# Roboy/gym-roboy

Measured on AMD Instinct MI355X. Metric: env-steps/sec, MsjRobot (3-DOF/8-tendon) batched rollout, higher is better.
Workload: dtype f32

## Files before the change

gym_roboy_amd/csrc/msj_kernels.hpp:

```cpp
#pragma once
#include "rtc_compat.hpp"
#include "msj_math.hpp"
#include "philox.hpp"
#include "env_common.hpp"

#if defined(RB_JIT_TABLE)
namespace rbk { __device__ constexpr rb::MsjConst<float, 8> BAKED = RB_JIT_TABLE; }
#else
#include "msj_baked.hpp"
#endif

namespace rbk {

using rbe::EnvParams;
using rbe::GoalBox;
using rbe::goal_value;
using rbe::mul_then_add;

constexpr int NT8 = 8;
constexpr int RS = rb::MsjModel<float, 8>::RS;
using Const8 = rb::MsjConst<float, NT8>;
constexpr int NTX = 16;
using ConstX = rb::MsjConst<float, NTX>;


template <bool BK, typename CONST>
__device__ __forceinline__ const CONST &robot_consts(const CONST &kernarg) {
    if constexpr (BK) return rbk::BAKED; else return kernarg;
}

struct SpLds {
    const float *col;
    int stride;
    __device__ __forceinline__ float operator()(int k) const { return col[k * stride]; }
};

struct Scale8 { float v[NT8]; };

template <int INTEG, int BLOCK, int UNROLL, bool BK = false>
__global__ void __launch_bounds__(BLOCK)
msj_step_env_per_lane(const Const8 c_arg, float *__restrict__ q, float *__restrict__ qd,
                      uint32_t *__restrict__ feas, const float *__restrict__ act, const Scale8 us, long n, long cnt) {
    const Const8 &c = robot_consts<BK>(c_arg);
    const long i = long(blockIdx.x) * BLOCK + threadIdx.x;
    if (i >= cnt) return;
    float qq[3], vv[3], sp[NT8];
    const float4 a0 = reinterpret_cast<const float4 *>(act)[2 * i];
    const float4 a1 = reinterpret_cast<const float4 *>(act)[2 * i + 1];
#pragma unroll
    for (int j = 0; j < 3; ++j) { qq[j] = q[j * n + i]; vv[j] = qd[j * n + i]; }
    const float a[NT8] = {a0.x, a0.y, a0.z, a0.w, a1.x, a1.y, a1.z, a1.w};
#pragma unroll
    for (int k = 0; k < NT8; ++k) sp[k] = a[k] * us.v[k];
    bool ok;
    if (UNROLL >= NT8) {
        ok = rb::MsjModel<float, NT8>::template step_sp<INTEG, UNROLL>(c, qq, vv, rb::SpArray<float, NT8>{sp});
    } else {
        __shared__ float lds_sp[NT8][BLOCK];
#pragma unroll
        for (int k = 0; k < NT8; ++k) lds_sp[k][threadIdx.x] = sp[k];
        ok = rb::MsjModel<float, NT8>::template step_sp<INTEG, UNROLL>(c, qq, vv, SpLds{&lds_sp[0][threadIdx.x], BLOCK});
    }
#pragma unroll
    for (int j = 0; j < 3; ++j) { q[j * n + i] = qq[j]; qd[j * n + i] = vv[j]; }
    feas[i] = ok ? 1u : 0u;
}




__device__ __forceinline__ __amdgpu_buffer_rsrc_t wg_rsrc(const void *base, int bytes) {
    return __builtin_amdgcn_make_buffer_rsrc(const_cast<void *>(base), 0, bytes, 0x00020000);
}

template <int INTEG, int BLOCK, bool BK = false>
__global__ void __launch_bounds__(BLOCK)
msj_step_env_per_lane_rs(const Const8 c_arg, float *__restrict__ q, float *__restrict__ qd,
                         uint32_t *__restrict__ feas, const float *__restrict__ act, const Scale8 us, long n, long cnt) {
    const Const8 &c = robot_consts<BK>(c_arg);
    const long env0 = long(blockIdx.x) * BLOCK;
    const long left = cnt - env0;
    const int live = int(left < BLOCK ? left : BLOCK);
    const int le = int(threadIdx.x);
    if (le >= live) return;
    const int off = le * 4;
    float qq[3], vv[3], u[NT8];
    const __amdgpu_buffer_rsrc_t ra = wg_rsrc(act + env0 * NT8, live * NT8 * 4);
    typedef float f4 __attribute__((ext_vector_type(4)));
    const f4 a0 = __builtin_bit_cast(f4, __builtin_amdgcn_raw_buffer_load_b128(ra, off * NT8, 0, 0));
    const f4 a1 = __builtin_bit_cast(f4, __builtin_amdgcn_raw_buffer_load_b128(ra, off * NT8 + 16, 0, 0));
#pragma unroll
    for (int j = 0; j < 3; ++j) {
        qq[j] = __uint_as_float(__builtin_amdgcn_raw_buffer_load_b32(wg_rsrc(q + j * n + env0, live * 4), off, 0, 0));
        vv[j] = __uint_as_float(__builtin_amdgcn_raw_buffer_load_b32(wg_rsrc(qd + j * n + env0, live * 4), off, 0, 0));
    }
    const float a[NT8] = {a0.x, a0.y, a0.z, a0.w, a1.x, a1.y, a1.z, a1.w};
#pragma unroll
    for (int k = 0; k < NT8; ++k) u[k] = a[k] * us.v[k];
    const bool ok = rb::MsjModel<float, NT8>::template step_rs<INTEG>(c, qq, vv, u);
#pragma unroll
    for (int j = 0; j < 3; ++j) {
        __builtin_amdgcn_raw_buffer_store_b32(__float_as_uint(qq[j]), wg_rsrc(q + j * n + env0, live * 4), off, 0, 0);
        __builtin_amdgcn_raw_buffer_store_b32(__float_as_uint(vv[j]), wg_rsrc(qd + j * n + env0, live * 4), off, 0, 0);
    }
    __builtin_amdgcn_raw_buffer_store_b32(ok ? 1u : 0u, wg_rsrc(feas + env0, live * 4), off, 0, 0);
}


struct PairMap { int a[4], d[4]; };
struct Scale4 { float v[4]; };

template <int CTRL>
__device__ __forceinline__ float rbk_dpp(float v) {
    return __int_as_float(__builtin_amdgcn_update_dpp(0, __float_as_int(v), CTRL, 0xF, 0xF, true));
}

template <int MIRROR>
struct AccelMirrorHalf {
    const Const8 &c;
    const float *u;
    __device__ __forceinline__ void operator()(const float q[3], const float qd[3], float qdd[3]) const {
        using M = rb::MsjModel<float, NT8>;
        const M::Frame f = M::frame(q, qd);
        float tx, ty, tz;
        M::half_torque(c, f, u, tx, ty, tz);
        M::template mirror_combine<MIRROR>(tx, ty, tz, rbk_dpp<0xB1>(tx), rbk_dpp<0xB1>(ty), rbk_dpp<0xB1>(tz));
        M::rigid_body(c, f, qd, tx, ty, tz, qdd);
    }
};

template <int INTEG, int BLOCK, int MIRROR, bool BK = false>
__global__ void __launch_bounds__(BLOCK)
msj_step_mirror_pairs(const Const8 c_arg, const PairMap pm, float *__restrict__ q, float *__restrict__ qd,
                      uint32_t *__restrict__ feas, const float *__restrict__ act, const Scale4 us, long n, long cnt) {
    const Const8 &c = robot_consts<BK>(c_arg);
    const long env0 = long(blockIdx.x) * (BLOCK / 2);
    const long left = cnt - env0;
    const int live = int(left < BLOCK / 2 ? left : BLOCK / 2);
    const int le = int(threadIdx.x >> 1);
    if (le >= live) return;
    const bool odd = (threadIdx.x & 1) != 0;
    const int off = le * 4, oddi = int(threadIdx.x & 1);
    float qq[3], vv[3], u[4];
    const __amdgpu_buffer_rsrc_t ra = wg_rsrc(act + env0 * NT8, live * NT8 * 4);
#pragma unroll
    for (int k = 0; k < 4; ++k) u[k] = __uint_as_float(__builtin_amdgcn_raw_buffer_load_b32(ra, off * NT8 + pm.a[k] + oddi * pm.d[k], 0, 0)) * us.v[k];
#pragma unroll
    for (int j = 0; j < 3; ++j) {
        qq[j] = __uint_as_float(__builtin_amdgcn_raw_buffer_load_b32(wg_rsrc(q + j * n + env0, live * 4), off, 0, 0));
        vv[j] = __uint_as_float(__builtin_amdgcn_raw_buffer_load_b32(wg_rsrc(qd + j * n + env0, live * 4), off, 0, 0));
    }
    constexpr int F0 = MIRROR == 0 ? 0 : 1, F1 = 2;
    const uint32_t flip = odd ? 0x80000000u : 0u;
    qq[F0] = __uint_as_float(__float_as_uint(qq[F0]) ^ flip); vv[F0] = __uint_as_float(__float_as_uint(vv[F0]) ^ flip);
    qq[F1] = __uint_as_float(__float_as_uint(qq[F1]) ^ flip); vv[F1] = __uint_as_float(__float_as_uint(vv[F1]) ^ flip);
    const bool ok = rb::MsjModel<float, NT8>::template integrate_acc<INTEG>(c, qq, vv, AccelMirrorHalf<MIRROR>{c, u});
    const int soff = odd ? 0x7fffff00 : le * 4;
#pragma unroll
    for (int j = 0; j < 3; ++j) {
        __builtin_amdgcn_raw_buffer_store_b32(__float_as_uint(qq[j]), wg_rsrc(q + j * n + env0, live * 4), soff, 0, 0);
        __builtin_amdgcn_raw_buffer_store_b32(__float_as_uint(vv[j]), wg_rsrc(qd + j * n + env0, live * 4), soff, 0, 0);
    }
    __builtin_amdgcn_raw_buffer_store_b32(ok ? 1u : 0u, wg_rsrc(feas + env0, live * 4), soff, 0, 0);
}


template <int INTEG, int BLOCK, int UNROLL, bool BK = false>
__global__ void __launch_bounds__(BLOCK)
msj_rollout_fused(const Const8 c_arg, float *__restrict__ q, float *__restrict__ qd, uint32_t *__restrict__ feas,
                  const float *__restrict__ act_ring, int ring, int n_steps, const Scale8 us, long n) {
    const Const8 &c = robot_consts<BK>(c_arg);
    const long i = long(blockIdx.x) * BLOCK + threadIdx.x;
    if (i >= n) return;
    float qq[3], vv[3];
#pragma unroll
    for (int j = 0; j < 3; ++j) { qq[j] = q[j * n + i]; vv[j] = qd[j * n + i]; }
    bool ok = true;
    const float4 *rec = reinterpret_cast<const float4 *>(act_ring) + 2 * i;
    float4 a0 = rec[0], a1 = rec[1];
    __shared__ float lds_sp[UNROLL >= NT8 ? 1 : NT8][BLOCK];
    int slab = 0;
    for (int t = 0; t < n_steps; ++t) {
        const float a[NT8] = {a0.x, a0.y, a0.z, a0.w, a1.x, a1.y, a1.z, a1.w};
        float sp[NT8];
#pragma unroll
        for (int k = 0; k < NT8; ++k) sp[k] = a[k] * us.v[k];
        if (t + 1 < n_steps) {
            slab = slab + 1 == ring ? 0 : slab + 1;
            const float4 *nx = rec + long(slab) * 2 * n;
            a0 = nx[0]; a1 = nx[1];
        }
        if (UNROLL == RS) {
            ok = rb::MsjModel<float, NT8>::template step_rs<INTEG>(c, qq, vv, sp);
        } else if (UNROLL >= NT8) {
            ok = rb::MsjModel<float, NT8>::template step_sp<INTEG, UNROLL>(c, qq, vv, rb::SpArray<float, NT8>{sp});
        } else {
#pragma unroll
            for (int k = 0; k < NT8; ++k) lds_sp[k][threadIdx.x] = sp[k];
            ok = rb::MsjModel<float, NT8>::template step_sp<INTEG, UNROLL>(c, qq, vv, SpLds{&lds_sp[0][threadIdx.x], BLOCK});
        }
    }
#pragma unroll
    for (int j = 0; j < 3; ++j) { q[j * n + i] = qq[j]; qd[j * n + i] = vv[j]; }
    feas[i] = ok ? 1u : 0u;
}



__device__ __forceinline__ void draw_goal3(const float (&lo)[3], const float (&hi)[3], uint64_t seed, uint64_t gid, uint32_t draw, float g[3]) {
    const rb::Philox4 r = rb::philox_draw(seed, gid, draw, rb::STREAM_GOALS, 0u);
#pragma unroll
    for (int j = 0; j < 3; ++j) g[j] = goal_value(lo[j], hi[j], r.v[j]);
}
__device__ __forceinline__ void draw_goal3(const GoalBox &box, uint64_t seed, uint64_t gid, uint32_t draw, float g[3]) {
    const float lo[3] = {box.lo[0], box.lo[1], box.lo[2]}, hi[3] = {box.hi[0], box.hi[1], box.hi[2]};
    draw_goal3(lo, hi, seed, gid, draw, g);
}

struct MsjEnvArgs {
    EnvParams e;
    float box_lo[3], box_hi[3];
    float *q, *qd;
    uint32_t *feas;
    float *goal;
    uint32_t *step_num;
    float *ep_ret;
    uint32_t *goal_count;
    const float *act;
    float *obs, *reward;
    uint32_t *done;
    double *ep_sum;
    uint32_t *ep_cnt, *infeas_n;
    long n, cnt;
    uint64_t seed, env0;
};
__host__ __device__ constexpr int msj_env_args_offset(int lead) { return (lead + int(alignof(MsjEnvArgs)) - 1) / int(alignof(MsjEnvArgs)) * int(alignof(MsjEnvArgs)); }
typedef const __attribute__((address_space(4))) MsjEnvArgs *msj_env_kernarg_ptr;
__device__ __forceinline__ msj_env_kernarg_ptr late_env_args(int offset) {
    const __attribute__((address_space(4))) char *p = (const __attribute__((address_space(4))) char *)__builtin_amdgcn_kernarg_segment_ptr();
    asm volatile("" : "+s"(p));
    return (msj_env_kernarg_ptr)(p + offset);
}

struct NoDoneHook {
    __device__ __forceinline__ void operator()(long, uint64_t, uint64_t, int) const {}
};

template <typename ARGS, typename HOOK = NoDoneHook>
__device__ __forceinline__ void env_account(ARGS a, long i, float (&qq)[3], float (&vv)[3], float (&gg)[3], bool ok,
                                            const HOOK &on_done = HOOK{}) {
    EnvParams e;
    e.vel_penalty = a->e.vel_penalty; e.bonus = a->e.bonus; e.max_len = a->e.max_len; e.auto_reset = a->e.auto_reset;
    e.penalty = a->e.penalty; e.bonus_val = a->e.bonus_val;
    e.a_lo = a->e.a_lo; e.a_hi = a->e.a_hi; e.v_lo = a->e.v_lo; e.v_hi = a->e.v_hi;
    e.act_hi = a->e.act_hi; e.slope = a->e.slope; e.tol_a2 = a->e.tol_a2; e.tol_v2 = a->e.tol_v2;
    e.a_scale = a->e.a_scale; e.v_scale = a->e.v_scale;
    const long n = a->n;
    float *__restrict__ q = a->q, *__restrict__ qd = a->qd, *__restrict__ goal = a->goal, *__restrict__ ep_ret = a->ep_ret;
    float *__restrict__ obs = a->obs, *__restrict__ reward = a->reward;
    uint32_t *__restrict__ feas = a->feas, *__restrict__ step_num = a->step_num, *__restrict__ goal_count = a->goal_count;
    uint32_t *__restrict__ done = a->done, *__restrict__ ep_cnt = a->ep_cnt, *__restrict__ infeas_n = a->infeas_n;
    double *__restrict__ ep_sum = a->ep_sum;
    uint32_t sn = step_num[i] + 1u;

    float dq2 = 0.0f, dv2 = 0.0f;
#pragma unroll
    for (int j = 0; j < 3; ++j) {
        const float dq = qq[j] - gg[j];
        dq2 += dq * dq;
        dv2 += vv[j] * vv[j];
    }
    bool reached;
    float r = rbe::env_reward(e, dq2, dv2, ok, reached);
    const bool dn = reached || (sn > uint32_t(e.max_len));

    float o[9] = {qq[0], qq[1], qq[2], vv[0], vv[1], vv[2], gg[0], gg[1], gg[2]};
    float ret = ep_ret[i] + r;
    uint32_t fz = ok ? 1u : 0u;
    if (!ok) infeas_n[i] += 1u;
    if (dn) {
        rbe::stat_add(&ep_sum[i], double(ret)); rbe::stat_add(&ep_sum[n + i], double(ret) * double(ret));
        rbe::stat_add(&ep_cnt[i], 1u); rbe::stat_add(&ep_cnt[n + i], sn - 1u); rbe::stat_add(&ep_cnt[2 * n + i], reached ? 1u : 0u);
        const uint64_t gid = a->env0 + uint64_t(i);
        const uint64_t seed = a->seed;
        const float lo[3] = {a->box_lo[0], a->box_lo[1], a->box_lo[2]}, hi[3] = {a->box_hi[0], a->box_hi[1], a->box_hi[2]};
        uint32_t draw = goal_count[i];
        draw_goal3(lo, hi, seed, gid, draw + (e.auto_reset ? 1u : 0u), gg);
        on_done(i, gid, seed, e.auto_reset);
        draw += e.auto_reset ? 2u : 1u;
        if (e.auto_reset) {
#pragma unroll
            for (int j = 0; j < 3; ++j) { qq[j] = 0.0f; vv[j] = 0.0f; o[j] = 0.0f; o[3 + j] = 0.0f; o[6 + j] = gg[j]; }
            sn = 1u; fz = 1u;
        }
        ret = 0.0f;
        goal_count[i] = draw;
#pragma unroll
        for (int j = 0; j < 3; ++j) goal[j * n + i] = gg[j];
    }
#pragma unroll
    for (int j = 0; j < 3; ++j) { q[j * n + i] = qq[j]; qd[j * n + i] = vv[j]; }
    feas[i] = fz; step_num[i] = sn; ep_ret[i] = ret;
    typedef float f4u __attribute__((ext_vector_type(4), aligned(4)));
    float *orow = obs + i * 9;
    *reinterpret_cast<f4u *>(orow) = f4u{o[0], o[1], o[2], o[3]};
    *reinterpret_cast<f4u *>(orow + 4) = f4u{o[4], o[5], o[6], o[7]};
    orow[8] = o[8];
    reward[i] = r; done[i] = dn ? 1u : 0u;
}

template <int INTEG, int BLOCK, int UNROLL, typename CONST = Const8, bool BK = false>
__global__ void __launch_bounds__(BLOCK)
msj_env_step_kernel(const CONST c_arg, const MsjEnvArgs a) {
    const float *__restrict__ q = a.q, *__restrict__ qd = a.qd, *__restrict__ goal = a.goal, *__restrict__ act = a.act;
    const long n = a.n, cnt = a.cnt;
    const float slope = a.e.slope, act_hi = a.e.act_hi;
    const CONST &c = robot_consts<BK>(c_arg);
    const long i = long(blockIdx.x) * BLOCK + threadIdx.x;
    if (i >= cnt) return;
    float qq[3], vv[3], gg[3];
#pragma unroll
    for (int j = 0; j < 3; ++j) { qq[j] = q[j * n + i]; vv[j] = qd[j * n + i]; gg[j] = goal[j * n + i]; }
    auto rescale = [&](float x) { return mul_then_add(slope, fminf(fmaxf(x, -1.0f), 1.0f) - 1.0f, act_hi); };
    bool ok;
    if constexpr (UNROLL == 0) {
        __shared__ float lds_sp[NTX][BLOCK];
        const int nt = c.nt;
        const float *row = act + i * nt;
        for (int k = 0; k < nt; ++k) lds_sp[k][threadIdx.x] = rescale(row[k]) * c.ten[k].ksg;
        ok = rb::MsjModel<float, NTX>::template step_sp<INTEG, 0>(c, qq, vv, SpLds{&lds_sp[0][threadIdx.x], BLOCK});
    } else {
    float sp[NT8];
    const float4 a0 = reinterpret_cast<const float4 *>(act)[2 * i];
    const float4 a1 = reinterpret_cast<const float4 *>(act)[2 * i + 1];
    const float av[NT8] = {a0.x, a0.y, a0.z, a0.w, a1.x, a1.y, a1.z, a1.w};
#pragma unroll
    for (int k = 0; k < NT8; ++k) sp[k] = rescale(av[k]) * c.ten[k].ksg;
    if (UNROLL == RS) {
        ok = rb::MsjModel<float, NT8>::template step_rs<INTEG>(c, qq, vv, sp);
    } else if (UNROLL >= NT8) {
        ok = rb::MsjModel<float, NT8>::template step_sp<INTEG, UNROLL>(c, qq, vv, rb::SpArray<float, NT8>{sp});
    } else {
        __shared__ float lds_sp[NT8][BLOCK];
#pragma unroll
        for (int k = 0; k < NT8; ++k) lds_sp[k][threadIdx.x] = sp[k];
        ok = rb::MsjModel<float, NT8>::template step_sp<INTEG, UNROLL>(c, qq, vv, SpLds{&lds_sp[0][threadIdx.x], BLOCK});
    }
    }
    if constexpr (BK) env_account(&a, i, qq, vv, gg, ok);
    else env_account(late_env_args(msj_env_args_offset(int(sizeof(CONST)))), i, qq, vv, gg, ok);
}


template <int INTEG, int BLOCK, int MIRROR, bool BK = false>
__global__ void __launch_bounds__(BLOCK)
msj_env_step_mirror_pairs(const Const8 c_arg, const PairMap pm, const MsjEnvArgs a) {
    const float *__restrict__ q = a.q, *__restrict__ qd = a.qd, *__restrict__ goal = a.goal, *__restrict__ act = a.act;
    const long n = a.n, cnt = a.cnt;
    const float slope = a.e.slope, act_hi = a.e.act_hi;
    const Const8 &c = robot_consts<BK>(c_arg);
    const long wg0 = long(blockIdx.x) * (BLOCK / 2);
    const long left = cnt - wg0;
    const int live = int(left < BLOCK / 2 ? left : BLOCK / 2);
    const int le = int(threadIdx.x >> 1);
    if (le >= live) return;
    const bool odd = (threadIdx.x & 1) != 0;
    const int off = le * 4, oddi = int(threadIdx.x & 1);
    const long i = wg0 + le;
    float qq[3], vv[3], gg[3], u[4];
    const __amdgpu_buffer_rsrc_t ra = wg_rsrc(act + wg0 * NT8, live * NT8 * 4);
#pragma unroll
    for (int k = 0; k < 4; ++k) {
        const float x = __uint_as_float(__builtin_amdgcn_raw_buffer_load_b32(ra, off * NT8 + pm.a[k] + oddi * pm.d[k], 0, 0));
        u[k] = mul_then_add(slope, fminf(fmaxf(x, -1.0f), 1.0f) - 1.0f, act_hi) * c.ten[k].ksg;
    }
#pragma unroll
    for (int j = 0; j < 3; ++j) {
        qq[j] = __uint_as_float(__builtin_amdgcn_raw_buffer_load_b32(wg_rsrc(q + j * n + wg0, live * 4), off, 0, 0));
        vv[j] = __uint_as_float(__builtin_amdgcn_raw_buffer_load_b32(wg_rsrc(qd + j * n + wg0, live * 4), off, 0, 0));
        gg[j] = __uint_as_float(__builtin_amdgcn_raw_buffer_load_b32(wg_rsrc(goal + j * n + wg0, live * 4), off, 0, 0));
    }
    constexpr int F0 = MIRROR == 0 ? 0 : 1, F1 = 2;
    const uint32_t flip = odd ? 0x80000000u : 0u;
    qq[F0] = __uint_as_float(__float_as_uint(qq[F0]) ^ flip); vv[F0] = __uint_as_float(__float_as_uint(vv[F0]) ^ flip);
    qq[F1] = __uint_as_float(__float_as_uint(qq[F1]) ^ flip); vv[F1] = __uint_as_float(__float_as_uint(vv[F1]) ^ flip);
    const bool ok = rb::MsjModel<float, NT8>::template integrate_acc<INTEG>(c, qq, vv, AccelMirrorHalf<MIRROR>{c, u});
    if (odd) return;
    if constexpr (BK) env_account(&a, i, qq, vv, gg, ok);
    else env_account(late_env_args(msj_env_args_offset(int(sizeof(Const8) + sizeof(PairMap)))), i, qq, vv, gg, ok);
}


}
```

gym_roboy_amd/csrc/msj_math.hpp:

```cpp
#pragma once
#include "rtc_compat.hpp"

#if defined(__HIPCC__)
#define RB_HD __host__ __device__ __forceinline__
#else
#define RB_HD inline
#endif


namespace rb {

template <typename T> struct Fast;
template <> struct Fast<double> {
    static RB_HD void sincos(double x, double &s, double &c) { s = ::sin(x); c = ::cos(x); }
    static RB_HD double exp(double x) { return ::exp(x); }
    static RB_HD double exp2(double x) { return ::exp2(x); }
    static RB_HD double rsqrt(double x) { return 1.0 / ::sqrt(x); }
    static RB_HD double rcp(double x) { return 1.0 / x; }
};
template <> struct Fast<float> {
    static RB_HD void sincos(float x, float &s, float &c) {
#if defined(__HIP_DEVICE_COMPILE__)
        s = __sinf(x); c = __cosf(x);
#else
        s = ::sinf(x); c = ::cosf(x);
#endif
    }
    static RB_HD float exp(float x) {
#if defined(__HIP_DEVICE_COMPILE__)
        return __expf(x);
#else
        return ::expf(x);
#endif
    }
    static RB_HD float exp2(float x) {
#if defined(__HIP_DEVICE_COMPILE__)
        return __builtin_amdgcn_exp2f(x);
#else
        return ::exp2f(x);
#endif
    }
    static RB_HD float rsqrt(float x) {
#if defined(__HIP_DEVICE_COMPILE__)
        return __builtin_amdgcn_rsqf(x);
#else
        return 1.0f / ::sqrtf(x);
#endif
    }
    static RB_HD float rcp(float x) {
#if defined(__HIP_DEVICE_COMPILE__)
        return __builtin_amdgcn_rcpf(x);
#else
        return 1.0f / x;
#endif
    }
};

template <typename T> RB_HD T tmin(T a, T b) {
#if defined(__HIP_DEVICE_COMPILE__)
    if constexpr (std::is_same<T, float>::value) return __builtin_fminf(a, b);
#endif
    return a < b ? a : b;
}
template <typename T> RB_HD T tmax(T a, T b) {
#if defined(__HIP_DEVICE_COMPILE__)
    if constexpr (std::is_same<T, float>::value) return __builtin_fmaxf(a, b);
#endif
    return a > b ? a : b;
}
template <typename T> RB_HD T tclamp(T x, T lo, T hi) {
#if defined(__HIP_DEVICE_COMPILE__)
    if constexpr (std::is_same<T, float>::value) return __builtin_amdgcn_fmed3f(x, lo, hi);
#endif
    return tmin(tmax(x, lo), hi);
}

template <typename T>
struct alignas(64) MsjTendon {
    T A[3];
    T Bv[3];
    T B2[3];
    T ab2;
    T il0s;
    T elcs;
    T ksg;
    T fmaxv;
    T pad[2];
};

template <typename T>
struct TendonUnits {
    T lc;
    T vl0;
    T fmax;
    T pad;
};

template <typename T>
struct TendonReading { T length, rate, activation, force; };

template <typename T, int NT>
struct MsjConst {
    MsjTendon<T> ten[NT];
    T IO[6];
    T mc[3];
    T g[3];
    T arm[3], damp[3], qlo[3], qhi[3], qdmax[3];
    T kps;
    T pe_k2s;
    T inv_pe_den;
    T fv_c1l, fv_c2l;
    T fv_c2s;
    T fv_k;
    T h;
    int32_t nsub;
    int32_t simple;
    int32_t nt;
};

template <typename T, int NT>
struct SpArray {
    const T *v;
    RB_HD T operator()(int k) const { return v[k]; }
};

struct NominalBody {
    template <typename T> RB_HD T mass(T x) const { return x; }
    template <typename T> RB_HD T damping(int, T x) const { return x; }
};

template <typename T, int NT>
struct MsjModel {
    using C = MsjConst<T, NT>;

    struct Frame {
        T s0, c0, s1, c1, s2, c2;
        T r00, r01, r02, r10, r11, r12, r20, r21, r22;
        T wx, wy, wz;
    };

    static RB_HD Frame frame(const T q[3], const T qd[3]) {
        Frame f;
        Fast<T>::sincos(q[0], f.s0, f.c0);
        Fast<T>::sincos(q[1], f.s1, f.c1);
        Fast<T>::sincos(q[2], f.s2, f.c2);
        f.r00 = f.c1 * f.c2; f.r01 = -f.c1 * f.s2; f.r02 = f.s1;
        f.r10 = f.c0 * f.s2 + f.s0 * f.s1 * f.c2; f.r11 = f.c0 * f.c2 - f.s0 * f.s1 * f.s2; f.r12 = -f.s0 * f.c1;
        f.r20 = f.s0 * f.s2 - f.c0 * f.s1 * f.c2; f.r21 = f.s0 * f.c2 + f.c0 * f.s1 * f.s2; f.r22 = f.c0 * f.c1;
        f.wx = f.r00 * qd[0] + f.s2 * qd[1];
        f.wy = f.r01 * qd[0] + f.c2 * qd[1];
        f.wz = f.r02 * qd[0] + qd[2];
        return f;
    }

    static RB_HD void tendon(const C &c, const Frame &f, const MsjTendon<T> &t, T u, T &tx, T &ty, T &tz) {
        const T ax = f.r00 * t.A[0] + f.r10 * t.A[1] + f.r20 * t.A[2];
        const T ay = f.r01 * t.A[0] + f.r11 * t.A[1] + f.r21 * t.A[2];
        const T az = f.r02 * t.A[0] + f.r12 * t.A[1] + f.r22 * t.A[2];
        const T d2 = ax * t.B2[0] + (ay * t.B2[1] + (az * t.B2[2] + t.ab2));
        const T mx = ay * t.Bv[2] - az * t.Bv[1];
        const T my = az * t.Bv[0] - ax * t.Bv[2];
        const T mz = ax * t.Bv[1] - ay * t.Bv[0];
        tendon_force(c, f, t, u, d2, mx, my, mz, tx, ty, tz);
    }

    static RB_HD void tendon_force(const C &c, const Frame &f, const MsjTendon<T> &t, T u, T d2, T mx, T my, T mz,
                                   T &tx, T &ty, T &tz) {
        const T inv = Fast<T>::rsqrt(d2);
        const T v = (f.wx * mx + f.wy * my + f.wz * mz) * inv;
        const T es = (d2 * inv) * t.il0s + t.elcs;
        const T act = tclamp(c.kps * es - u, T(0), T(1));
        const T fl = Fast<T>::exp2(-(es * es));
        const T vp = tmax(v, T(0)), p = tclamp(v + T(1), T(0), T(1));
        const T num = c.fv_c1l * vp + p;
        const T den = c.fv_c2l * vp + (c.fv_c2s * p + c.fv_k);
        const T rden = Fast<T>::rcp(den);
        const T fpe = tmax(Fast<T>::exp2(c.pe_k2s * es) * c.inv_pe_den - c.inv_pe_den, T(0));
        const T Fs = (t.fmaxv * inv) * ((act * fl) * num * rden + fpe);
        tx -= Fs * mx; ty -= Fs * my; tz -= Fs * mz;
    }

    static RB_HD TendonReading<T> tendon_state(const C &c, const Frame &f, const MsjTendon<T> &t, const TendonUnits<T> &pu, T u) {
        const T ax = f.r00 * t.A[0] + f.r10 * t.A[1] + f.r20 * t.A[2];
        const T ay = f.r01 * t.A[0] + f.r11 * t.A[1] + f.r21 * t.A[2];
        const T az = f.r02 * t.A[0] + f.r12 * t.A[1] + f.r22 * t.A[2];
        const T d2 = ax * t.B2[0] + (ay * t.B2[1] + (az * t.B2[2] + t.ab2));
        const T mx = ay * t.Bv[2] - az * t.Bv[1];
        const T my = az * t.Bv[0] - ax * t.Bv[2];
        const T mz = ax * t.Bv[1] - ay * t.Bv[0];
        const T inv = Fast<T>::rsqrt(d2);
        const T v = (f.wx * mx + f.wy * my + f.wz * mz) * inv;
        const T dl = d2 * inv;
        const T es = dl * t.il0s + t.elcs;
        const T act = tclamp(c.kps * es - u, T(0), T(1));
        const T fl = Fast<T>::exp2(-(es * es));
        const T vp = tmax(v, T(0)), p = tclamp(v + T(1), T(0), T(1));
        const T num = c.fv_c1l * vp + p;
        const T den = c.fv_c2l * vp + (c.fv_c2s * p + c.fv_k);
        const T rden = Fast<T>::rcp(den);
        const T fpe = tmax(Fast<T>::exp2(c.pe_k2s * es) * c.inv_pe_den - c.inv_pe_den, T(0));
        TendonReading<T> r;
        r.length = dl + pu.lc;
        r.rate = v * pu.vl0;
        r.activation = act;
        r.force = pu.fmax * ((act * fl) * num * rden + fpe);
        return r;
    }

    static RB_HD MsjTendon<T> scaled_tendon(const MsjTendon<T> &t, T fscale) {
        MsjTendon<T> s = t;
        s.fmaxv = t.fmaxv * fscale;
        return s;
    }

    static RB_HD T prescale(const C &c, int k, T setpoint) { return c.ten[k].ksg * setpoint; }

    template <typename BP> static RB_HD T bmass(const BP *bp, T x) {
        if constexpr (std::is_same<BP, NominalBody>::value) return x; else return bp->mass(x);
    }
    template <typename BP> static RB_HD T bdamp(const BP *bp, int j, T x) {
        if constexpr (std::is_same<BP, NominalBody>::value) return x; else return bp->damping(j, x);
    }
    template <typename BP = NominalBody>
    static RB_HD void rigid_body(const C &c, const Frame &f, const T qd[3], T tx, T ty, T tz, T qdd[3], const BP *bp = nullptr) {
        const T r00 = f.r00, r01 = f.r01, r02 = f.r02, s2 = f.s2, c2 = f.c2;
        const T Ixx = bmass(bp, c.IO[0]), Iyy = bmass(bp, c.IO[1]), Izz = bmass(bp, c.IO[2]);
        const T z0x = -f.s1 * c2 * qd[1] - f.c1 * s2 * qd[2];
        const T z0y = f.s1 * s2 * qd[1] - f.c1 * c2 * qd[2];
        const T z0z = f.c1 * qd[1];
        const T bx = z0x * qd[0] + c2 * qd[2] * qd[1];
        const T by = z0y * qd[0] - s2 * qd[2] * qd[1];
        const T bz = z0z * qd[0];
        T m00, m01, m02, m11, m12, m22, vx, vy, vz;
        if (c.simple) {
            const T a0x = Ixx * r00, a0y = Iyy * r01, a0z = Izz * r02;
            const T a1x = Ixx * s2, a1y = Iyy * c2;
            m00 = r00 * a0x + r01 * a0y + r02 * a0z + c.arm[0];
            m01 = s2 * a0x + c2 * a0y;
            m02 = a0z;
            m11 = s2 * a1x + c2 * a1y + c.arm[1];
            m12 = T(0);
            m22 = Izz + c.arm[2];
            const T hx = Ixx * f.wx, hy = Iyy * f.wy, hz = Izz * f.wz;
            const T nx = Ixx * bx + (f.wy * hz - f.wz * hy);
            const T ny = Iyy * by + (f.wz * hx - f.wx * hz);
            const T nz = Izz * bz + (f.wx * hy - f.wy * hx);
            const T k = bmass(bp, c.mc[2]) * c.g[2];
            vx = tx - k * f.r21 - nx;
            vy = ty + k * f.r20 - ny;
            vz = tz - nz;
        } else {
            const T Ixy = bmass(bp, c.IO[3]), Ixz = bmass(bp, c.IO[4]), Iyz = bmass(bp, c.IO[5]);
            const T a0x = Ixx * r00 + Ixy * r01 + Ixz * r02;
            const T a0y = Ixy * r00 + Iyy * r01 + Iyz * r02;
            const T a0z = Ixz * r00 + Iyz * r01 + Izz * r02;
            const T a1x = Ixx * s2 + Ixy * c2;
            const T a1y = Ixy * s2 + Iyy * c2;
            const T a1z = Ixz * s2 + Iyz * c2;
            m00 = r00 * a0x + r01 * a0y + r02 * a0z + c.arm[0];
            m01 = s2 * a0x + c2 * a0y;
            m02 = a0z;
            m11 = s2 * a1x + c2 * a1y + c.arm[1];
            m12 = a1z;
            m22 = Izz + c.arm[2];
            const T hx = a0x * qd[0] + a1x * qd[1] + Ixz * qd[2];
            const T hy = a0y * qd[0] + a1y * qd[1] + Iyz * qd[2];
            const T hz = a0z * qd[0] + a1z * qd[1] + Izz * qd[2];
            const T nx = Ixx * bx + Ixy * by + Ixz * bz + (f.wy * hz - f.wz * hy);
            const T ny = Ixy * bx + Iyy * by + Iyz * bz + (f.wz * hx - f.wx * hz);
            const T nz = Ixz * bx + Iyz * by + Izz * bz + (f.wx * hy - f.wy * hx);
            const T gx = r00 * c.g[0] + f.r10 * c.g[1] + f.r20 * c.g[2];
            const T gy = r01 * c.g[0] + f.r11 * c.g[1] + f.r21 * c.g[2];
            const T gz = r02 * c.g[0] + f.r12 * c.g[1] + f.r22 * c.g[2];
            vx = tx + (bmass(bp, c.mc[1]) * gz - bmass(bp, c.mc[2]) * gy) - nx;
            vy = ty + (bmass(bp, c.mc[2]) * gx - bmass(bp, c.mc[0]) * gz) - ny;
            vz = tz + (bmass(bp, c.mc[0]) * gy - bmass(bp, c.mc[1]) * gx) - nz;
        }
        const T t0 = r00 * vx + r01 * vy + r02 * vz - bdamp(bp, 0, c.damp[0]) * qd[0];
        const T t1 = s2 * vx + c2 * vy - bdamp(bp, 1, c.damp[1]) * qd[1];
        const T t2 = vz - bdamp(bp, 2, c.damp[2]) * qd[2];
        const T k00 = m11 * m22 - m12 * m12;
        const T k01 = m02 * m12 - m01 * m22;
        const T k02 = m01 * m12 - m02 * m11;
        const T k11 = m00 * m22 - m02 * m02;
        const T k12 = m01 * m02 - m00 * m12;
        const T k22 = m00 * m11 - m01 * m01;
        const T idet = Fast<T>::rcp(m00 * k00 + m01 * k01 + m02 * k02);
        qdd[0] = (k00 * t0 + k01 * t1 + k02 * t2) * idet;
        qdd[1] = (k01 * t0 + k11 * t1 + k12 * t2) * idet;
        qdd[2] = (k02 * t0 + k12 * t1 + k22 * t2) * idet;
    }

    template <int UNROLL, typename SP>
    struct AccelAllTendons {
        const C &c;
        const SP &sp;
        RB_HD void operator()(const T q[3], const T qd[3], T qdd[3]) const {
            const Frame f = frame(q, qd);
            T tx = T(0), ty = T(0), tz = T(0);
            if (UNROLL == 0) {
#pragma unroll 1
                for (int k = 0; k < c.nt; ++k) tendon(c, f, c.ten[k], sp(k), tx, ty, tz);
            } else {
                constexpr int U = UNROLL > 0 ? UNROLL : 1;
#pragma unroll U
                for (int k = 0; k < NT; ++k) tendon(c, f, c.ten[k], sp(k), tx, ty, tz);
            }
            rigid_body(c, f, qd, tx, ty, tz, qdd);
        }
    };

    template <int MIRROR> static RB_HD T mirror_sign(int j) { return (j == 2 || j == MIRROR) ? T(-1) : T(1); }
    static RB_HD void half_torque(const C &c, const Frame &f, const T u[4], T &tx, T &ty, T &tz) {
        tx = T(0); ty = T(0); tz = T(0);
#pragma unroll
        for (int k = 0; k < 4; ++k) {
            tendon(c, f, c.ten[k], u[k], tx, ty, tz);
#if defined(__HIP_DEVICE_COMPILE__)
            __builtin_amdgcn_sched_barrier(0);
#endif
        }
    }
    template <int MIRROR>
    static RB_HD void mirror_combine(T &tx, T &ty, T &tz, T px, T py, T pz) {
        tx = MIRROR == 0 ? tx - px : tx + px;
        ty = MIRROR == 0 ? ty + py : ty - py;
        tz = tz - pz;
    }

    static RB_HD void sat(const C &c, const T v[3], T out[3]) {
#pragma unroll
        for (int j = 0; j < 3; ++j) out[j] = tclamp(v[j], -c.qdmax[j], c.qdmax[j]);
    }

    static RB_HD bool limit(const C &c, T q[3], T qd[3]) {
        bool ok = true;
#pragma unroll
        for (int j = 0; j < 3; ++j) {
            const bool over = q[j] > c.qhi[j], under = q[j] < c.qlo[j];
            qd[j] = tclamp(qd[j], under ? T(0) : -c.qdmax[j], over ? T(0) : c.qdmax[j]);
            q[j] = tclamp(q[j], c.qlo[j], c.qhi[j]);
            ok = ok && !(over || under);
        }
        return ok;
    }

    template <int INTEG, typename ACCEL>
    static RB_HD bool integrate(const C &c, T q[3], T qd[3], const ACCEL &accel) {
        bool feasible = true;
        const T h = c.h;
        for (int sub = 0; sub < c.nsub; ++sub) {
            if (INTEG == 0) {
                T a[3];
                accel(q, qd, a);
#pragma unroll
                for (int j = 0; j < 3; ++j) {
                    qd[j] = tclamp(qd[j] + h * a[j], -c.qdmax[j], c.qdmax[j]);
                    q[j] = q[j] + h * qd[j];
                }
            } else {
                T k1q[3], k1v[3], k2q[3], k2v[3], k3q[3], k3v[3], k4q[3], k4v[3], qs[3], vs[3];
                const T hh = T(0.5) * h;
                sat(c, qd, k1q);
                accel(q, k1q, k1v);
#pragma unroll
                for (int j = 0; j < 3; ++j) { qs[j] = q[j] + hh * k1q[j]; vs[j] = qd[j] + hh * k1v[j]; }
                sat(c, vs, k2q);
                accel(qs, k2q, k2v);
#pragma unroll
                for (int j = 0; j < 3; ++j) { qs[j] = q[j] + hh * k2q[j]; vs[j] = qd[j] + hh * k2v[j]; }
                sat(c, vs, k3q);
                accel(qs, k3q, k3v);
#pragma unroll
                for (int j = 0; j < 3; ++j) { qs[j] = q[j] + h * k3q[j]; vs[j] = qd[j] + h * k3v[j]; }
                sat(c, vs, k4q);
                accel(qs, k4q, k4v);
                const T h6 = h * T(1.0 / 6.0);
#pragma unroll
                for (int j = 0; j < 3; ++j) {
                    q[j] = q[j] + h6 * (k1q[j] + T(2) * k2q[j] + T(2) * k3q[j] + k4q[j]);
                    qd[j] = qd[j] + h6 * (k1v[j] + T(2) * k2v[j] + T(2) * k3v[j] + k4v[j]);
                }
            }
            feasible = limit(c, q, qd) && feasible;
        }
        return feasible;
    }

    template <int INTEG, typename ACCEL>
    static RB_HD bool integrate_acc(const C &c, T q[3], T qd[3], const ACCEL &accel) {
        if (INTEG == 0) return integrate<0>(c, q, qd, accel);
        bool feasible = true;
        const T h = c.h, h6 = c.h * T(1.0 / 6.0);
        for (int sub = 0; sub < c.nsub; ++sub) {
            T aq[3] = {T(0), T(0), T(0)}, av[3] = {T(0), T(0), T(0)}, qs[3], vs[3];
#pragma unroll
            for (int j = 0; j < 3; ++j) { qs[j] = q[j]; vs[j] = qd[j]; }
#pragma unroll 1
            for (int stage = 0; stage < 4; ++stage) {
                T kq[3], kv[3];
                sat(c, vs, kq);
                accel(qs, kq, kv);
                const T w = (stage == 0 || stage == 3) ? T(1) : T(2);
                const T a = stage < 2 ? T(0.5) * h : h;
#pragma unroll
                for (int j = 0; j < 3; ++j) {
                    aq[j] += w * kq[j]; av[j] += w * kv[j];
                    qs[j] = q[j] + a * kq[j]; vs[j] = qd[j] + a * kv[j];
                }
            }
#pragma unroll
            for (int j = 0; j < 3; ++j) { q[j] = q[j] + h6 * aq[j]; qd[j] = qd[j] + h6 * av[j]; }
            feasible = limit(c, q, qd) && feasible;
        }
        return feasible;
    }

    struct AccelPinned {
        const C &c;
        const T *u;
        RB_HD void operator()(const T q[3], const T qd[3], T qdd[3]) const {
            const Frame f = frame(q, qd);
            T tx = T(0), ty = T(0), tz = T(0);
#pragma unroll
            for (int k = 0; k < NT; ++k) {
                tendon(c, f, c.ten[k], u[k], tx, ty, tz);
#if defined(__HIP_DEVICE_COMPILE__)
                __builtin_amdgcn_sched_barrier(0);
#endif
            }
            rigid_body(c, f, qd, tx, ty, tz, qdd);
        }
    };
    static constexpr int RS = 9;
    template <int INTEG>
    static RB_HD bool step_rs(const C &c, T q[3], T qd[3], const T u[NT]) {
        return integrate_acc<INTEG>(c, q, qd, AccelPinned{c, u});
    }

    template <int INTEG, int UNROLL, typename SP>
    static RB_HD bool step_sp(const C &c, T q[3], T qd[3], const SP &sp) {
        return integrate<INTEG>(c, q, qd, AccelAllTendons<UNROLL, SP>{c, sp});
    }

    template <int INTEG, int UNROLL = NT>
    static RB_HD bool step(const C &c, T q[3], T qd[3], const T sp[NT]) {
        T u[NT];
#pragma unroll
        for (int k = 0; k < NT; ++k) u[k] = prescale(c, k, sp[k]);
        const SpArray<T, NT> src{u};
        return step_sp<INTEG, UNROLL>(c, q, qd, src);
    }
};

}
```

Baseline: 19.00 billion.

## Pair tendon evaluation with pinned schedule and spill two activations to LDS

Replaces the per-tendon pinned accelerator with a paired version that interleaves routing, strain, Hill and torque stages of two tendons between scheduling barriers, so transcendental latency can overlap. It also keeps six scaled activations in registers and parks the last two in shared memory, reading them back on each evaluation. The aim is to lower register pressure for occupancy while keeping ILP. The cost is extra LDS traffic and interleaved live ranges that may raise register use again.

Result: faster. 20.40 billion, median of 6 (+7.4%).

```diff
diff --git a/gym_roboy_amd/csrc/msj_kernels.hpp b/gym_roboy_amd/csrc/msj_kernels.hpp
--- a/gym_roboy_amd/csrc/msj_kernels.hpp
+++ b/gym_roboy_amd/csrc/msj_kernels.hpp
@@ -33,6 +33,14 @@
     const float *col;
     int stride;
     __device__ __forceinline__ float operator()(int k) const { return col[k * stride]; }
+};
+
+template <int KEEP>
+struct SpSplit {
+    const float *reg;
+    const float *col;
+    int stride;
+    __device__ __forceinline__ float operator()(int k) const { return k < KEEP ? reg[k] : col[(k - KEEP) * stride]; }
 };
 
 struct Scale8 { float v[NT8]; };
@@ -97,7 +105,11 @@
     const float a[NT8] = {a0.x, a0.y, a0.z, a0.w, a1.x, a1.y, a1.z, a1.w};
 #pragma unroll
     for (int k = 0; k < NT8; ++k) u[k] = a[k] * us.v[k];
-    const bool ok = rb::MsjModel<float, NT8>::template step_rs<INTEG>(c, qq, vv, u);
+    constexpr int KEEP = NT8 - 2;
+    __shared__ float lds_u[NT8 - KEEP][BLOCK];
+#pragma unroll
+    for (int k = KEEP; k < NT8; ++k) lds_u[k - KEEP][le] = u[k];
+    const bool ok = rb::MsjModel<float, NT8>::template step_rs_paired<INTEG>(c, qq, vv, SpSplit<KEEP>{u, &lds_u[0][le], BLOCK});
 #pragma unroll
     for (int j = 0; j < 3; ++j) {
         __builtin_amdgcn_raw_buffer_store_b32(__float_as_uint(qq[j]), wg_rsrc(q + j * n + env0, live * 4), off, 0, 0);
diff --git a/gym_roboy_amd/csrc/msj_math.hpp b/gym_roboy_amd/csrc/msj_math.hpp
--- a/gym_roboy_amd/csrc/msj_math.hpp
+++ b/gym_roboy_amd/csrc/msj_math.hpp
@@ -432,12 +432,96 @@
             rigid_body(c, f, qd, tx, ty, tz, qdd);
         }
     };
+
+    struct Routing { T d2, mx, my, mz; };
+    static RB_HD Routing routing(const Frame &f, const MsjTendon<T> &t) {
+        const T ax = f.r00 * t.A[0] + f.r10 * t.A[1] + f.r20 * t.A[2];
+        const T ay = f.r01 * t.A[0] + f.r11 * t.A[1] + f.r21 * t.A[2];
+        const T az = f.r02 * t.A[0] + f.r12 * t.A[1] + f.r22 * t.A[2];
+        Routing r;
+        r.d2 = ax * t.B2[0] + (ay * t.B2[1] + (az * t.B2[2] + t.ab2));
+        r.mx = ay * t.Bv[2] - az * t.Bv[1];
+        r.my = az * t.Bv[0] - ax * t.Bv[2];
+        r.mz = ax * t.Bv[1] - ay * t.Bv[0];
+        return r;
+    }
+    struct Strain { T v, es, fl, pe; };
+    static RB_HD Strain strain(const C &c, const Frame &f, const MsjTendon<T> &t, const Routing &r, T inv) {
+        Strain s;
+        s.v = (f.wx * r.mx + f.wy * r.my + f.wz * r.mz) * inv;
+        s.es = (r.d2 * inv) * t.il0s + t.elcs;
+        s.fl = Fast<T>::exp2(-(s.es * s.es));
+        s.pe = Fast<T>::exp2(c.pe_k2s * s.es);
+        return s;
+    }
+    struct Hill { T afn, rden; };
+    static RB_HD Hill hill(const C &c, const Strain &s, T u) {
+        const T act = tclamp(c.kps * s.es - u, T(0), T(1));
+        const T vp = tmax(s.v, T(0)), p = tclamp(s.v + T(1), T(0), T(1));
+        const T num = c.fv_c1l * vp + p;
+        const T den = c.fv_c2l * vp + (c.fv_c2s * p + c.fv_k);
+        Hill h;
+        h.rden = Fast<T>::rcp(den);
+        h.afn = (act * s.fl) * num;
+        return h;
+    }
+    static RB_HD void torque(const C &c, const MsjTendon<T> &t, const Routing &r, T inv, const Strain &s, const Hill &h,
+                             T &tx, T &ty, T &tz) {
+        const T fpe = tmax(s.pe * c.inv_pe_den - c.inv_pe_den, T(0));
+        const T Fs = (t.fmaxv * inv) * (h.afn * h.rden + fpe);
+        tx -= Fs * r.mx; ty -= Fs * r.my; tz -= Fs * r.mz;
+    }
+    static RB_HD void pin() {
+#if defined(__HIP_DEVICE_COMPILE__)
+        __builtin_amdgcn_sched_barrier(0);
+#endif
+    }
+    static RB_HD void tendon_pair(const C &c, const Frame &f, const MsjTendon<T> &ta, const MsjTendon<T> &tb, T ua, T ub,
+                                  T &tx, T &ty, T &tz) {
+        const Routing ra = routing(f, ta);
+        pin();
+        const T ia = Fast<T>::rsqrt(ra.d2);
+        const Routing rb_ = routing(f, tb);
+        pin();
+        const T ib = Fast<T>::rsqrt(rb_.d2);
+        const Strain sa = strain(c, f, ta, ra, ia);
+        pin();
+        const Hill ha = hill(c, sa, ua);
+        const Strain sb = strain(c, f, tb, rb_, ib);
+        pin();
+        torque(c, ta, ra, ia, sa, ha, tx, ty, tz);
+        const Hill hb = hill(c, sb, ub);
+        pin();
+        torque(c, tb, rb_, ib, sb, hb, tx, ty, tz);
+        pin();
+    }
+    template <typename SP>
+    struct AccelPaired {
+        const C &c;
+        const SP &sp;
+        RB_HD void operator()(const T q[3], const T qd[3], T qdd[3]) const {
+            static_assert(NT % 2 == 0, "tendons in pairs");
+            const Frame f = frame(q, qd);
+            T tx = T(0), ty = T(0), tz = T(0);
+#pragma unroll
+            for (int k = 0; k < NT; k += 2) {
+                const T ua = sp(k), ub = sp(k + 1);
+                tendon_pair(c, f, c.ten[k], c.ten[k + 1], ua, ub, tx, ty, tz);
+            }
+            rigid_body(c, f, qd, tx, ty, tz, qdd);
+        }
+    };
     static constexpr int RS = 9;
     template <int INTEG>
     static RB_HD bool step_rs(const C &c, T q[3], T qd[3], const T u[NT]) {
         return integrate_acc<INTEG>(c, q, qd, AccelPinned{c, u});
     }
 
+    template <int INTEG, typename SP>
+    static RB_HD bool step_rs_paired(const C &c, T q[3], T qd[3], const SP &sp) {
+        return integrate_acc<INTEG>(c, q, qd, AccelPaired<SP>{c, sp});
+    }
+
     template <int INTEG, int UNROLL, typename SP>
     static RB_HD bool step_sp(const C &c, T q[3], T qd[3], const SP &sp) {
         return integrate<INTEG>(c, q, qd, AccelAllTendons<UNROLL, SP>{c, sp});
```
